# NoahVl/Explaining-In-Style-Reproducibility-Study

Measured on AMD Instinct MI355X. Metric: StylEx G+D+enc train-step images/sec @256px, higher is better.
Workload: dtype bf16; 1 GPU; FFHQ-shaped 256x256 StylEx, batch 32/GPU, GAE=2 (noise+encoder micro-steps), GP every 4th step, ResNet-18 classifier; image_size=256, batch_per_gpu=32, start_step=0, gradient_accumulate_every=2, global_batch=32, parallelism=dp1

## Files before the change

explaining-in-style-reproducibility-study_amd/csrc/fused_bwd.hip:

```cpp
#include <hip/hip_runtime.h>
#include <stdint.h>

#include "stylex_internal.h"

namespace {

constexpr int NT = 256;

template <int K>
struct Acc {
    float4 v[K];
    __device__ __forceinline__ void zero() {
#pragma unroll
        for (int k = 0; k < K; ++k) v[k] = make_float4(0.f, 0.f, 0.f, 0.f);
    }
};

template <int K>
__device__ __forceinline__ void block_reduce_store(Acc<K>& a, float* smem, int cv, int prow, int CV, int rpp, int C,
                                                   float* partial_row , bool active) {
    float4* s4 = reinterpret_cast<float4*>(smem);
    if (active) {
#pragma unroll
        for (int k = 0; k < K; ++k) s4[(k * rpp + prow) * CV + cv] = a.v[k];
    }
    __syncthreads();
    if (active && prow == 0) {
#pragma unroll
        for (int k = 0; k < K; ++k) {
            float4 t = make_float4(0.f, 0.f, 0.f, 0.f);
            for (int r = 0; r < rpp; ++r) {
                float4 u = s4[(k * rpp + r) * CV + cv];
                t.x += u.x; t.y += u.y; t.z += u.z; t.w += u.w;
            }
            float* d = partial_row + (long)k * C + cv * 4;
            if (cv * 4 + 3 < C) {
                *reinterpret_cast<float4*>(d) = t;
            } else {
                float tt[4] = {t.x, t.y, t.z, t.w};
                for (int e = 0; e < 4 && cv * 4 + e < C; ++e) d[e] = tt[e];
            }
        }
    }
}

struct Geo {
    int b, cv, prow, CV, rpp;
    long p_begin, p_end;
    bool active;
};

__device__ __forceinline__ Geo make_geo(int HW, int C, int nchunks) {
    Geo g;
    g.CV = (C + 3) / 4;
    if (g.CV > NT) g.CV = NT;
    g.rpp = NT / g.CV;
    g.cv = threadIdx.x % g.CV;
    g.prow = threadIdx.x / g.CV;
    g.active = g.prow < g.rpp;
    g.b = blockIdx.y;
    long per = ((long)HW + nchunks - 1) / nchunks;
    g.p_begin = (long)blockIdx.x * per;
    g.p_end = g.p_begin + per < HW ? g.p_begin + per : HW;
    return g;
}

__device__ __forceinline__ float4 ld4(const void* p, long off, int bf) { return act_ld4(p, off, bf); }
__device__ __forceinline__ void st4(void* p, long off, float4 v, int bf) { act_st4(p, off, v, bf); }
__device__ __forceinline__ float4 ldp4(const float* p) { return *reinterpret_cast<const float4*>(p); }

__global__ __launch_bounds__(NT) void act_bwd_reduce_kernel(const void* __restrict__ dy, const void* __restrict__ y,
                                                           void* __restrict__ dx, float* __restrict__ partial, int HW,
                                                           int C, int nchunks, int lrelu, float scale, int bf) {
    extern __shared__ __attribute__((aligned(16))) float smem[];
    Geo g = make_geo(HW, C, nchunks);
    Acc<1> a;
    a.zero();
    const int c = g.cv * 4;
    if (g.active && c < C) {
        const long base = (long)g.b * HW;
        for (long p = g.p_begin + g.prow; p < g.p_end; p += g.rpp) {
            const long o = (base + p) * C + c;
            float4 gv = ld4(dy, o, bf);
            gv.x *= scale; gv.y *= scale; gv.z *= scale; gv.w *= scale;
            if (lrelu) {
                const float slope = lrelu == 2 ? 0.f : 0.2f;
                float4 yv = ld4(y, o, bf);
                gv.x = yv.x > 0.f ? gv.x : slope * gv.x;
                gv.y = yv.y > 0.f ? gv.y : slope * gv.y;
                gv.z = yv.z > 0.f ? gv.z : slope * gv.z;
                gv.w = yv.w > 0.f ? gv.w : slope * gv.w;
            }
// ... 62 lines not shown
    extern __shared__ __attribute__((aligned(16))) float smem[];
    Geo g = make_geo(HW, C, nchunks);
    Acc<1> a;
    a.zero();
    const int c = g.cv * 4;
    if (g.active && c < C) {
        float4 s4 = ldp4(s + (long)g.b * C + c);
        const long base = (long)g.b * HW;
        for (long p = g.p_begin + g.prow; p < g.p_end; p += g.rpp) {
            const long o = (base + p) * C + c;
            float4 tv = ld4(t, o, bf);
            float4 xv = ld4(x, o, bf);
            a.v[0].x += xv.x * tv.x; a.v[0].y += xv.y * tv.y; a.v[0].z += xv.z * tv.z; a.v[0].w += xv.w * tv.w;
            if (gx) {
                tv.x *= s4.x; tv.y *= s4.y; tv.z *= s4.z; tv.w *= s4.w;
                st4(gx, o, tv, bf);
            }
        }
    }
    block_reduce_store<1>(a, smem, g.cv, g.prow, g.CV, g.rpp, C, partial + ((long)g.b * nchunks + blockIdx.x) * C,
                          g.active && c < C);
}

inline size_t reduce_smem(int C, int K) {
    int CV = (C + 3) / 4;
    if (CV > NT) CV = NT;
    int rpp = NT / CV;
    return (size_t)K * rpp * CV * 16;
}

inline bool ok_shape(const int64_t* sh, int nchunks) {
    return sh[0] > 0 && sh[1] > 0 && sh[2] > 0 && sh[3] > 0 && sh[3] <= 1024 && (sh[3] % 4 == 0) && nchunks > 0 &&
           sh[0] <= 65535;
}

}

extern "C" {

int stylex_reduce_chunks(const int64_t* sh) {
    long HW = (long)sh[1] * sh[2];
    long n = (2048 + sh[0] - 1) / sh[0];
    long maxc = (HW + 63) / 64;
    if (n > maxc) n = maxc;
    if (n < 1) n = 1;
    return (int)n;
}

int stylex_act_bwd_reduce(const void* dy, const void* y, void* dx, float* partial, const int64_t* sh, int nchunks,
                          int lrelu, float scale, int act_dtype, void* stream) {
    if (act_dtype != 0 && act_dtype != 1) return STYLEX_EINVAL;
    if (!dy || !partial || !ok_shape(sh, nchunks) || (lrelu && !y)) return STYLEX_EINVAL;
    int HW = (int)(sh[1] * sh[2]), C = (int)sh[3];
    hipLaunchKernelGGL(act_bwd_reduce_kernel, dim3(nchunks, (unsigned)sh[0]), dim3(NT), reduce_smem(C, 1),
                       (hipStream_t)stream, dy, y, dx, partial, HW, C, nchunks, lrelu, scale, act_dtype);
    return (int)hipGetLastError();
}

// ... 44 lines not shown
```

explaining-in-style-reproducibility-study_amd/stylex/hip_backend.py:

```python
import os as _os

if _os.environ.get("STYLEX_MIOPEN_ALLOW_BWD_GTC", "0") != "1":
    _os.environ.setdefault("MIOPEN_DEBUG_CONV_IMPLICIT_GEMM_ASM_BWD_GTC_XDLOPS_NHWC", "0")

import atexit
import ctypes
import os
import weakref

import torch

_HERE = os.path.dirname(os.path.abspath(__file__))
LIB_PATH = os.path.join(os.path.dirname(_HERE), "libstylex_hip.so")

F32, BF16, BF16_ACT = 0, 1, 2
EPI_BIAS, EPI_LRELU, EPI_OSCALE, EPI_NOISE, EPI_RESIDUAL, EPI_RELU, EPI_GATE, EPI_NOISE_NAT = 1, 2, 4, 8, 16, 32, 64, 128
EPI_MASK_OUT, EPI_GATE_MASK = 256, 512

_c_f = ctypes.c_void_p
_i64p = ctypes.POINTER(ctypes.c_int64)


class ConvEpilogue(ctypes.Structure):
    _fields_ = [
# ... 42 lines not shown
    "stylex_fold_weight_grad_s2d": (ctypes.c_int, [_c_f, _c_f, _i64p, ctypes.c_void_p]),
    "stylex_conv2d_bwd_weight_s2d_supported": (ctypes.c_int, [_i64p, ctypes.c_int, ctypes.c_int]),
    "stylex_conv2d_bwd_weight_s2d": (ctypes.c_int, [ctypes.c_void_p, ctypes.c_void_p, _c_f, ctypes.c_void_p, ctypes.c_int64, _i64p,
                                                    ctypes.c_int, ctypes.c_float, ctypes.c_int, ctypes.c_int, ctypes.c_void_p]),
    "stylex_upsample2x_bilinear_fwd": (ctypes.c_int, [_c_f, _c_f, _i64p, ctypes.c_int, ctypes.c_void_p]),
    "stylex_upsample2x_bilinear_bwd": (ctypes.c_int, [_c_f, _c_f, _i64p, ctypes.c_int, ctypes.c_void_p]),
    "stylex_rgb_up_blur_add_fwd": (ctypes.c_int, [_c_f, _c_f, _c_f, _i64p, ctypes.c_int, ctypes.c_void_p]),
    "stylex_rgb_up_blur_add_bwd": (ctypes.c_int, [_c_f, _c_f, _i64p, ctypes.c_int, ctypes.c_void_p]),
    "stylex_blur3x3_reflect_fwd": (ctypes.c_int, [_c_f, _c_f, _i64p, ctypes.c_int, ctypes.c_void_p]),
    "stylex_blur3x3_reflect_bwd": (ctypes.c_int, [_c_f, _c_f, _i64p, ctypes.c_int, ctypes.c_void_p]),
    "stylex_bias_act_fwd": (ctypes.c_int, [_c_f, _c_f, _c_f, ctypes.c_int64, _c_f, _c_f, _c_f, _i64p, ctypes.c_int,
                                           ctypes.c_void_p]),
    "stylex_bias_act_bwd": (ctypes.c_int, [_c_f, _c_f, _c_f, _i64p, ctypes.c_int, ctypes.c_void_p]),
    "stylex_rowwise_sumsq": (ctypes.c_int, [_c_f, _c_f, _i64p, ctypes.c_void_p]),
    "stylex_reduce_chunks": (ctypes.c_int, [_i64p]),
    "stylex_act_bwd_reduce": (ctypes.c_int, [_c_f, _c_f, _c_f, _c_f, _i64p, ctypes.c_int, ctypes.c_int, ctypes.c_float,
                                             ctypes.c_int, ctypes.c_void_p]),
    "stylex_modconv_bwd_prep": (ctypes.c_int, [_c_f, _c_f, _c_f, ctypes.c_int64, _c_f, _c_f, _c_f, _c_f, _i64p,
                                               ctypes.c_int, ctypes.c_int, ctypes.c_int, ctypes.c_void_p]),
    "stylex_modconv_bwd_prep_scaled": (ctypes.c_int, [_c_f, _c_f, _c_f, ctypes.c_int64, _c_f, _c_f, _c_f, _c_f, _c_f, _i64p,
                                                      ctypes.c_int, ctypes.c_int, ctypes.c_int, ctypes.c_void_p]),
    "stylex_scale_reduce": (ctypes.c_int, [_c_f, _c_f, _c_f, _c_f, _c_f, _i64p, ctypes.c_int, ctypes.c_int,
                                           ctypes.c_void_p]),
    "stylex_pad_rgb8": (ctypes.c_int, [_c_f, _c_f, _i64p, _i64p, ctypes.c_int, ctypes.c_void_p]),
    "stylex_affine_act_nchw_fwd": (ctypes.c_int, [_c_f, _c_f, _c_f, _c_f, _c_f, ctypes.c_int64, ctypes.c_int64, ctypes.c_int64,
                                                  ctypes.c_int, ctypes.c_void_p]),
    "stylex_affine_act_nchw_bwd": (ctypes.c_int, [_c_f, _c_f, _c_f, _c_f, _c_f, ctypes.c_int64, ctypes.c_int64, ctypes.c_int64,
                                                  ctypes.c_int, ctypes.c_void_p]),
    "stylex_affine_relu_maxpool_fwd": (ctypes.c_int, [_c_f, _c_f, _c_f, _c_f, _c_f, ctypes.c_int64, ctypes.c_int64,
                                                      ctypes.c_int64, ctypes.c_int64, ctypes.c_void_p]),
    "stylex_affine_relu_maxpool_bwd": (ctypes.c_int, [_c_f, _c_f, _c_f, _c_f, ctypes.c_int64, ctypes.c_int64, ctypes.c_int64,
                                                      ctypes.c_int64, ctypes.c_void_p]),
    "stylex_lpips_tap_nhwc_fwd": (ctypes.c_int, [_c_f, _c_f, _c_f, _c_f, _c_f, _c_f, ctypes.c_int64, ctypes.c_int64, ctypes.c_int64,
                                                 ctypes.c_int64, ctypes.c_void_p]),
    "stylex_lpips_tap_nhwc_bwd": (ctypes.c_int, [_c_f, _c_f, _c_f, _c_f, _c_f, _c_f, _c_f, _c_f, ctypes.c_int64, ctypes.c_int64,
                                                 ctypes.c_int64, ctypes.c_void_p]),
    "stylex_nchw_f32_to_nhwc_bf16": (ctypes.c_int, [_c_f, _c_f, ctypes.c_int64, ctypes.c_int64, ctypes.c_int64, ctypes.c_int,
                                                    ctypes.c_void_p]),
    "stylex_nhwc_bf16_to_nchw_f32": (ctypes.c_int, [_c_f, _c_f, _c_f, ctypes.c_int64, ctypes.c_int64, ctypes.c_int64, ctypes.c_void_p]),
    "stylex_resize_norm_fwd": (ctypes.c_int, [_c_f, _c_f, _c_f, _c_f, _i64p, _i64p, ctypes.c_void_p]),
    "stylex_resize_norm_bwd": (ctypes.c_int, [_c_f, _c_f, _c_f, _i64p, ctypes.c_void_p]),
    "stylex_relu_gate_add": (ctypes.c_int, [_c_f, _c_f, _c_f, _c_f, ctypes.c_int64, ctypes.c_void_p]),
    "stylex_maxpool3s2_nhwc_fwd": (ctypes.c_int, [_c_f, _c_f, _c_f, _i64p, ctypes.c_void_p]),
    "stylex_maxpool3s2_nhwc_bwd": (ctypes.c_int, [_c_f, _c_f, _c_f, _i64p, ctypes.c_void_p]),
    "stylex_conv_image_grad": (ctypes.c_int, [_c_f, _c_f, _c_f, _i64p, ctypes.c_void_p]),
    "stylex_lpips_tap_fwd": (ctypes.c_int, [_c_f, _c_f, _c_f, _c_f, _c_f, _c_f, ctypes.c_int64, ctypes.c_int64, ctypes.c_int64,
# ... 1368 lines not shown
                                           _ptr(partial), shp, nch, lr, _adt(gy), _stream()), "stylex_modconv_bwd_prep")
    else:
        gz_scale = _f32(gz_scale)
        _check(lib.stylex_modconv_bwd_prep_scaled(_ptr(gy), _ptr(y), _ptr(noise), ns, _ptr(noise_w), _ptr(noise_b),
                                                  _ptr(gz_scale), _ptr(gz), _ptr(partial), shp, nch, lr, _adt(gy), _stream()),
               "stylex_modconv_bwd_prep_scaled")
    return gz, partial.sum(dim=1)


def scale_reduce(x, t, s, want_gx=True):
    lib = _ensure_device(x)
    assert is_cl(x) and is_cl(t) and x.dtype == t.dtype
    b, c, h, w = x.shape
    shp = _shape(b, h, w, c)
    nch = lib.stylex_reduce_chunks(shp)
    partial = _empty((b, nch, c), dtype=torch.float32, device=x.device)
    gx = empty_cl(tuple(x.shape), x) if want_gx else None
    s = _f32(s)
    _check(lib.stylex_scale_reduce(_ptr(x), _ptr(t), _ptr(s), _ptr(gx), _ptr(partial), shp, nch, _adt(x), _stream()),
           "stylex_scale_reduce")
    return gx, partial.sum(dim=1)


def torgb_ok(x):
    c = x.shape[1]
    if os.environ.get("STYLEX_TORGB", "1") == "0":
        return False
    return x.is_cuda and x.dtype == torch.bfloat16 and 8 <= c <= 512 and (c & (c - 1)) == 0


def torgb_fwd(x, s1, w):
    lib = _ensure_device(x)
    assert is_cl(x) and x.dtype == torch.bfloat16
    b, c, h, wd = x.shape
    y = empty_cl((b, 4, h, wd), x)
    s1, w = _f32(s1), _f32(w)
    _check(lib.stylex_torgb_fwd(_ptr(x), _ptr(s1), _ptr(w), _ptr(y), _shape(b, h, wd, c), _stream()), "stylex_torgb_fwd")
    return y


def torgb_bwd(x, gy, s1, w, want_gx=True):
    lib = _ensure_device(x)
    assert is_cl(x) and is_cl(gy) and gy.shape[1] == 4 and x.dtype == gy.dtype == torch.bfloat16
    b, c, h, wd = x.shape
    shp = _shape(b, h, wd, c)
    nch = lib.stylex_torgb_chunks(shp)
    partial = _empty((b, nch, 3, c), dtype=torch.float32, device=x.device)
    gx = empty_cl(tuple(x.shape), x) if want_gx else None
# ... 76 lines not shown
```

explaining-in-style-reproducibility-study_amd/stylex/networks.py:

```python
import atexit
import math
from math import log2

import os

import torch
import torch.nn.functional as F
from torch import nn

import ops


def exists(v):
    return v is not None


_SIDE = {}
atexit.register(_SIDE.clear)


def _side_stream(t, which=0):
    import os

    if not t.is_cuda or os.environ.get("STYLEX_STREAMS", "1") == "0":
# ... 83 lines not shown

class Conv2DMod(nn.Module):
    def __init__(self, in_chan, out_chan, kernel, demod=True, stride=1, dilation=1, eps=1e-8, **kwargs):
        super().__init__()
        assert stride == 1 and dilation == 1, "only the configuration the reference uses is implemented"
        self.filters, self.demod, self.kernel = out_chan, demod, kernel
        self.stride, self.dilation, self.eps = stride, dilation, eps
        self.weight = nn.Parameter(torch.randn((out_chan, in_chan, kernel, kernel)))
        nn.init.kaiming_normal_(self.weight, a=0, mode="fan_in", nonlinearity="leaky_relu")

    def forward(self, x, y):
        return ops.modulated_conv2d(x, y, self.weight, demod=self.demod, eps=self.eps)


class RGBBlock(nn.Module):
    def __init__(self, latent_dim, input_channel, upsample, rgba=False):
        super().__init__()
        self.input_channel = input_channel
        self.to_style = nn.Linear(latent_dim, input_channel)
        self.conv = Conv2DMod(input_channel, 4 if rgba else 3, 1, demod=False)
        self.upsample = nn.Sequential(Upsample2x(), Blur()) if upsample else None

    def forward(self, x, prev_rgb, istyle, style=None, padded=False):
        style = self.to_style(istyle) if style is None else style
        if padded and not self.conv.demod:
            fused = ops.rgb_block(x, prev_rgb, style, self.conv.weight, exists(self.upsample))
            if fused is not None:
                return fused
        if exists(prev_rgb) and prev_rgb.shape[1] == 4 and self.conv.weight.shape[0] == 3:
            prev_rgb = prev_rgb[:, :3]
        x = self.conv(x, style)
        if exists(prev_rgb):
            x = x + prev_rgb
        if exists(self.upsample):
            x = self.upsample(x)
        return x


class GeneratorBlock(nn.Module):
    def __init__(self, latent_dim, input_channels, filters, upsample=True, upsample_rgb=True, rgba=False):
        super().__init__()
        self.input_channels, self.filters = input_channels, filters
        self.num_style_coords = input_channels + filters
        self.upsample = Upsample2x() if upsample else None
        self.to_style1 = nn.Linear(latent_dim, input_channels)
        self.to_noise1 = nn.Linear(1, filters)
        self.conv1 = Conv2DMod(input_channels, filters, 3)
        self.to_style2 = nn.Linear(latent_dim, filters)
        self.to_noise2 = nn.Linear(1, filters)
        self.conv2 = Conv2DMod(filters, filters, 3)
        self.activation = leaky_relu()
        self.to_rgb = RGBBlock(latent_dim, filters, upsample_rgb, rgba)

    def forward_main(self, x, istyle, inoise, styles=None):
        if exists(self.upsample):
            x = self.upsample(x)
        coords = None
        self._rgb_style = None
        if styles is None:
            fused = ops.style_affines(istyle, self.to_style1, self.to_style2, self.to_rgb.to_style, self.__dict__.setdefault("_aff_cache", {}))
            if fused is not None:
                style1, style2, self._rgb_style, coords = fused
            else:
                style1, style2 = self.to_style1(istyle), self.to_style2(istyle)
        else:
            style1, style2 = styles
        x = ops.modconv_noise_act(x, style1, self.conv1.weight, inoise, self.to_noise1.weight[:, 0],
                                  self.to_noise1.bias, demod=self.conv1.demod, eps=self.conv1.eps)
        x = ops.modconv_noise_act(x, style2, self.conv2.weight, inoise, self.to_noise2.weight[:, 0],
                                  self.to_noise2.bias, demod=self.conv2.demod, eps=self.conv2.eps)
        return x, (coords if coords is not None else torch.cat([style1, style2], dim=-1))

    def forward(self, x, prev_rgb, istyle, inoise):
        x, coords = self.forward_main(x, istyle, inoise)
        rgb = self.to_rgb(x, prev_rgb, istyle, style=self.__dict__.pop("_rgb_style", None))
        return x, rgb, coords


class DiscriminatorBlock(nn.Module):
    def __init__(self, input_channels, filters, downsample=True):
        super().__init__()
        self.conv_res = HipConv2d(input_channels, filters, 1, stride=(2 if downsample else 1))
        self.net = nn.Sequential(HipConv2d(input_channels, filters, 3, padding=1, act=True), _FusedAct(),
                                 HipConv2d(filters, filters, 3, padding=1, act=True), _FusedAct())
        self.downsample = nn.Sequential(Blur(), HipConv2d(filters, filters, 3, padding=1, stride=2)) if downsample else None

    def forward(self, x):
        fused = getattr(ops.impl(), "dblock", None)
        if fused is not None:
# ... 98 lines not shown
```

explaining-in-style-reproducibility-study_amd/stylex/ops.py:

```python
import math

import os

import torch
from contextlib import nullcontext as _nullcontext
import torch.nn.functional as F

import hip_backend as hb

_PRECISION = hb.F32


_NAMES = {"fp32": hb.F32, "f32": hb.F32, "bf16": hb.BF16_ACT, "bf16_f32act": hb.BF16}


def set_precision(name):
    global _PRECISION
    _PRECISION = _NAMES[name]


def get_precision():
    return {hb.F32: "fp32", hb.BF16_ACT: "bf16", hb.BF16: "bf16_f32act"}[_PRECISION]


# ... 523 lines not shown
    @torch.autograd.function.once_differentiable
    def backward(ctx, gy):
        x, s1, w = ctx.saved_tensors
        gx, t = hb.torgb_bwd(x, _cl(gy), s1, w, want_gx=ctx.needs_input_grad[0])
        gs1 = gw = None
        if ctx.needs_input_grad[1]:
            gs1 = (t * w.reshape(1, 3, -1).float()).sum(dim=1)
        if ctx.needs_input_grad[2]:
            gw = (t * s1.float()[:, None, :]).sum(dim=0).reshape(w.shape).to(w.dtype)
        return gx, gs1, gw


class _RGBTailFast(torch.autograd.Function):

    @staticmethod
    def forward(ctx, rgb, prev):
        return hb.rgb_up_blur_add_fwd(_cl(rgb), _cl(prev) if prev is not None else None)

    @staticmethod
    @torch.autograd.function.once_differentiable
    def backward(ctx, gy):
        g = hb.rgb_up_blur_add_bwd(_cl(gy))
        return g, (g if ctx.needs_input_grad[1] else None)


class _BlurS2D(torch.autograd.Function):

    @staticmethod
    def forward(ctx, x):
        return hb.blur3x3_s2d_fwd(_cl(x))

    @staticmethod
    def backward(ctx, gy2):
        return _BlurS2DBwd.apply(gy2)


class _BlurS2DBwd(torch.autograd.Function):
    @staticmethod
    def forward(ctx, gy2):
        return hb.blur3x3_s2d_bwd(_cl(gy2))

    @staticmethod
    def backward(ctx, ggx):
        return _BlurS2D.apply(ggx)


# ... 419 lines not shown
        return _BiasAct.apply(_act(x + n), None)

    @staticmethod
    def upsample2x(x):
        return _Up.apply(_act(x))

    @staticmethod
    def blur3x3(x):
        return _Blur.apply(_act(x))

    @staticmethod
    def blur_down(x, weight, bias, residual, res_scale):
        b, c, h, w = x.shape
        if (_PRECISION != hb.F32 and c % 64 == 0 and weight.shape[0] % 4 == 0 and h % 2 == 0
                and w % 2 == 0 and w // 2 >= 16 and h // 2 >= 16 and tuple(weight.shape[2:]) == (3, 3)):
            x2 = _BlurS2D.apply(_act(x))
            if fast_enabled():
                return _DownS2DFast.apply(x2, weight, bias, _act(residual), res_scale)
            return _ConvBiasActDD.apply(x2, weight, bias, _act(residual), 1, 1, False, res_scale, c)
        return HipOps.conv2d(HipOps.blur3x3(x), weight, bias, stride=2, padding=1, residual=residual,
                             res_scale=res_scale)

    @staticmethod
    def rgb_block(x, prev_rgb, style, weight, upsample):
        if not fast_enabled() or os.environ.get("STYLEX_RGB_TAIL", "1") == "0":
            return None
        x = _act(x)
        if tuple(weight.shape[2:]) != (1, 1) or weight.shape[0] != 3 or not hb.torgb_ok(x):
            return None
        if prev_rgb is not None and (prev_rgb.shape[1] != 4 or prev_rgb.dtype != x.dtype):
            return None
        rgb = _ToRGBFast.apply(x, style + 1, weight)
        if upsample:
            return _RGBTailFast.apply(rgb, prev_rgb)
        return rgb if prev_rgb is None else rgb + prev_rgb

    @staticmethod
    def residual_merge(x, res):
        return (x + res) * (1 / math.sqrt(2))

    @staticmethod
    def dblock(x, conv_res, conv1, conv2, down):
        if not fast_enabled() or os.environ.get("STYLEX_DBLOCK", "1") == "0":
            return None
        if conv1.weight.shape[0] % 4 != 0:
            return None
        return _DBlockFast.apply(x, conv_res.weight, conv_res.bias, conv1.weight, conv1.bias, conv2.weight, conv2.bias,
                                 down.weight if down is not None else None, down.bias if down is not None else None,
                                 down is not None)

    @staticmethod
    def rowwise_sumsq(x2d):
        return _RowSumSq.apply(x2d)


_IMPL = HipOps


def use_impl(impl):
    global _IMPL
    prev = _IMPL
    _IMPL = impl
    return prev


def impl():
    return _IMPL


class _EqualLinearFast(torch.autograd.Function):

    @staticmethod
# ... 149 lines not shown
```

include/stylex_hip.h:

```cpp
#ifndef STYLEX_HIP_H
#define STYLEX_HIP_H

#include <stdint.h>

#ifdef __cplusplus
extern "C" {
#endif

#define STYLEX_F32 0
#define STYLEX_BF16 1
#define STYLEX_BF16_ACT 2

#define STYLEX_EINVAL (-1)
#define STYLEX_EWORKSPACE (-2)

#define STYLEX_CONV_NSHAPE 11

#define STYLEX_EPI_BIAS 1
#define STYLEX_EPI_LRELU 2
#define STYLEX_EPI_OSCALE 4
#define STYLEX_EPI_NOISE 8
#define STYLEX_EPI_RESIDUAL 16
#define STYLEX_EPI_RELU 32
#define STYLEX_EPI_NOISE_NAT 128
// ... 116 lines not shown
                              int64_t C, int64_t HW, int64_t partial_stride, void* stream);
int stylex_lpips_tap_nhwc_bwd(const void* f0, const void* f1, const float* lin, const float* r0, const float* r1, const float* gout,
                              void* g0, void* g1, int64_t B, int64_t C, int64_t HW, void* stream);

int stylex_weight_sumsq(const float* w, float* wsq, int64_t O, int64_t C, int64_t K, void* stream);
int stylex_modcoeff_fwd(const float* style, const float* wsq, float* s1, float* d, int64_t B, int64_t C, int64_t O,
                        float eps, void* stream);
int stylex_modcoeff_bwd(const float* gd, const float* d, const float* s1, const float* wsq, const float* w,
                        const float* gs1, float* gstyle, float* gw, int64_t B, int64_t C, int64_t O, int64_t K,
                        void* stream);

int stylex_reduce_chunks(const int64_t* shape);
int stylex_act_bwd_reduce(const void* dy, const void* y, void* dx, float* partial, const int64_t* shape, int nchunks,
                          int lrelu, float scale, int act_dtype, void* stream);
int stylex_modconv_bwd_prep(const void* gy, const void* y, const float* noise, int64_t noise_stride,
                            const float* noise_w, const float* noise_b, void* gz, float* partial,
                            const int64_t* shape, int nchunks, int lrelu, int act_dtype, void* stream);
int stylex_modconv_bwd_prep_scaled(const void* gy, const void* y, const float* noise, int64_t noise_stride,
                                   const float* noise_w, const float* noise_b, const float* gz_scale, void* gz,
                                   float* partial, const int64_t* shape, int nchunks, int lrelu, int act_dtype,
                                   void* stream);
int stylex_scale_reduce(const void* x, const void* t, const float* s, void* gx, float* partial, const int64_t* shape,
                        int nchunks, int act_dtype, void* stream);

int stylex_torgb_chunks(const int64_t* shape);
int stylex_torgb_fwd(const void* x, const float* s1, const float* w, void* y, const int64_t* shape, void* stream);
int stylex_torgb_bwd(const void* x, const void* gy, const float* s1, const float* w, void* gx, float* partial,
                     const int64_t* shape, void* stream);

int stylex_timing_enable(int on);
int stylex_timing_pause(int on);
int stylex_timing_report(int kernel_class, int64_t* launches, double* total_ms, double* total_flops,
                         double* total_bytes);
int stylex_timing_layers(int64_t* meta, double* vals, int64_t cap);
int stylex_timing_kernels(char* names, int64_t* meta, double* vals, int64_t cap);

#define STYLEX_ADAM_COPY_PACK 0
#define STYLEX_ADAM_COPY_PACK_S2D 1
#define STYLEX_ADAM_COPY_SUMSQ 2
typedef struct {
    float* p;
    const float* g;
    float* m;
    float* v;
    const float* step;
    int64_t numel;
// ... 32 lines not shown
```

Before: 992.0 images/sec.

## Fuse StyleGAN generator block forward/backward into custom autograd with fused backward kernels

Adds a fused generator-block autograd function that runs upsample, two modulated convs with noise/lrelu epilogues, and toRGB in one unit. Its backward uses two new HIP kernels that fold the RGB gradient, the incoming gradient sum, the lrelu backward, the noise weight/bias reductions and the demod-coefficient reductions into single passes over activations. The per-strip reduction helpers move into a shared header. This aims to cut separate elementwise and reduction kernels and repeated activation reads in generator backward, at the cost of saving more intermediates and adding extra code paths with shape guards.

```diff
diff --git a/explaining-in-style-reproducibility-study_amd/csrc/fused_bwd.hip b/explaining-in-style-reproducibility-study_amd/csrc/fused_bwd.hip
--- a/explaining-in-style-reproducibility-study_amd/csrc/fused_bwd.hip
+++ b/explaining-in-style-reproducibility-study_amd/csrc/fused_bwd.hip
@@ -2,72 +2,11 @@
 #include <stdint.h>
 
 #include "stylex_internal.h"
+#include "strip_reduce.h"
 
 namespace {
 
-constexpr int NT = 256;
-
-template <int K>
-struct Acc {
-    float4 v[K];
-    __device__ __forceinline__ void zero() {
-#pragma unroll
-        for (int k = 0; k < K; ++k) v[k] = make_float4(0.f, 0.f, 0.f, 0.f);
-    }
-};
-
-template <int K>
-__device__ __forceinline__ void block_reduce_store(Acc<K>& a, float* smem, int cv, int prow, int CV, int rpp, int C,
-                                                   float* partial_row , bool active) {
-    float4* s4 = reinterpret_cast<float4*>(smem);
-    if (active) {
-#pragma unroll
-        for (int k = 0; k < K; ++k) s4[(k * rpp + prow) * CV + cv] = a.v[k];
-    }
-    __syncthreads();
-    if (active && prow == 0) {
-#pragma unroll
-        for (int k = 0; k < K; ++k) {
-            float4 t = make_float4(0.f, 0.f, 0.f, 0.f);
-            for (int r = 0; r < rpp; ++r) {
-                float4 u = s4[(k * rpp + r) * CV + cv];
-                t.x += u.x; t.y += u.y; t.z += u.z; t.w += u.w;
-            }
-            float* d = partial_row + (long)k * C + cv * 4;
-            if (cv * 4 + 3 < C) {
-                *reinterpret_cast<float4*>(d) = t;
-            } else {
-                float tt[4] = {t.x, t.y, t.z, t.w};
-                for (int e = 0; e < 4 && cv * 4 + e < C; ++e) d[e] = tt[e];
-            }
-        }
-    }
-}
-
-struct Geo {
-    int b, cv, prow, CV, rpp;
-    long p_begin, p_end;
-    bool active;
-};
-
-__device__ __forceinline__ Geo make_geo(int HW, int C, int nchunks) {
-    Geo g;
-    g.CV = (C + 3) / 4;
-    if (g.CV > NT) g.CV = NT;
-    g.rpp = NT / g.CV;
-    g.cv = threadIdx.x % g.CV;
-    g.prow = threadIdx.x / g.CV;
-    g.active = g.prow < g.rpp;
-    g.b = blockIdx.y;
-    long per = ((long)HW + nchunks - 1) / nchunks;
-    g.p_begin = (long)blockIdx.x * per;
-    g.p_end = g.p_begin + per < HW ? g.p_begin + per : HW;
-    return g;
-}
-
-__device__ __forceinline__ float4 ld4(const void* p, long off, int bf) { return act_ld4(p, off, bf); }
-__device__ __forceinline__ void st4(void* p, long off, float4 v, int bf) { act_st4(p, off, v, bf); }
-__device__ __forceinline__ float4 ldp4(const float* p) { return *reinterpret_cast<const float4*>(p); }
+using namespace stylex_strip;
 
 __global__ __launch_bounds__(NT) void act_bwd_reduce_kernel(const void* __restrict__ dy, const void* __restrict__ y,
                                                            void* __restrict__ dx, float* __restrict__ partial, int HW,
@@ -176,18 +115,6 @@
                           g.active && c < C);
 }
 
-inline size_t reduce_smem(int C, int K) {
-    int CV = (C + 3) / 4;
-    if (CV > NT) CV = NT;
-    int rpp = NT / CV;
-    return (size_t)K * rpp * CV * 16;
-}
-
-inline bool ok_shape(const int64_t* sh, int nchunks) {
-    return sh[0] > 0 && sh[1] > 0 && sh[2] > 0 && sh[3] > 0 && sh[3] <= 1024 && (sh[3] % 4 == 0) && nchunks > 0 &&
-           sh[0] <= 65535;
-}
-
 }
 
 extern "C" {
diff --git a/explaining-in-style-reproducibility-study_amd/csrc/gblock_bwd.hip b/explaining-in-style-reproducibility-study_amd/csrc/gblock_bwd.hip
--- /dev/null
+++ b/explaining-in-style-reproducibility-study_amd/csrc/gblock_bwd.hip
@@ -0,0 +1,231 @@
+#include <hip/hip_runtime.h>
+#include <stdint.h>
+
+#include "stylex_internal.h"
+#include "strip_reduce.h"
+
+namespace {
+
+using namespace stylex_strip;
+
+__device__ __forceinline__ float4 rnd4(float4 v, int bf) { return bf ? act_unpack4(act_pack4(v)) : v; }
+
+__device__ __forceinline__ float noise_at(const float* noise, int ns, int natural, int b, int p, int W) {
+    const int h = p / W, w = p - h * W;
+    return natural ? noise[((long)b * ns + h) * ns + w] : noise[((long)b * ns + w) * ns + h];
+}
+
+__device__ __forceinline__ void prep_step(float4 gv, float4 yv, float nz, float4 w4, float4 b4, float4 d4, int lrelu,
+                                          bool scaled, void* gz, long o, int bf, float4* a) {
+    float4 t = yv;
+    if (lrelu) {
+        gv.x = yv.x > 0.f ? gv.x : 0.2f * gv.x; t.x = yv.x > 0.f ? yv.x : 5.f * yv.x;
+        gv.y = yv.y > 0.f ? gv.y : 0.2f * gv.y; t.y = yv.y > 0.f ? yv.y : 5.f * yv.y;
+        gv.z = yv.z > 0.f ? gv.z : 0.2f * gv.z; t.z = yv.z > 0.f ? yv.z : 5.f * yv.z;
+        gv.w = yv.w > 0.f ? gv.w : 0.2f * gv.w; t.w = yv.w > 0.f ? yv.w : 5.f * yv.w;
+    }
+    if (scaled) st4(gz, o, make_float4(gv.x * d4.x, gv.y * d4.y, gv.z * d4.z, gv.w * d4.w), bf);
+    else st4(gz, o, gv, bf);
+    a[0].x += gv.x * (t.x - (nz * w4.x + b4.x));
+    a[0].y += gv.y * (t.y - (nz * w4.y + b4.y));
+    a[0].z += gv.z * (t.z - (nz * w4.z + b4.z));
+    a[0].w += gv.w * (t.w - (nz * w4.w + b4.w));
+    a[1].x += gv.x * nz; a[1].y += gv.y * nz; a[1].z += gv.z * nz; a[1].w += gv.w * nz;
+    a[2].x += gv.x; a[2].y += gv.y; a[2].z += gv.z; a[2].w += gv.w;
+}
+
+template <bool RGB, bool BF>
+__global__ __launch_bounds__(NT) void gblock_out_bwd_kernel(const void* __restrict__ y, const void* __restrict__ ga,
+                                                           const void* __restrict__ gb, const void* __restrict__ grgb,
+                                                           const float* __restrict__ s_rgb, const float* __restrict__ w_rgb,
+                                                           const float* __restrict__ noise, int ns, int natural,
+                                                           const float* __restrict__ nw, const float* __restrict__ nb,
+                                                           const float* __restrict__ gz_scale, void* __restrict__ gz,
+                                                           float* __restrict__ partial, int H, int W, int C, int nchunks,
+                                                           int lrelu) {
+    extern __shared__ __attribute__((aligned(16))) float smem[];
+    constexpr int K = 3, bf = BF ? 1 : 0;
+    const int HW = H * W;
+    Geo g = make_geo(HW, C, nchunks);
+    Acc<K> a;
+    a.zero();
+    const int c = g.cv * 4;
+    if (g.active && c < C) {
+        float4 w4 = make_float4(0.f, 0.f, 0.f, 0.f), b4 = w4;
+        if (noise) {
+            w4 = ldp4(nw + c);
+            b4 = ldp4(nb + c);
+        }
+        float4 d4 = make_float4(1.f, 1.f, 1.f, 1.f);
+        if (gz_scale) d4 = ldp4(gz_scale + (long)g.b * C + c);
+        float4 m0 = w4, m1 = w4, m2 = w4;
+        if (RGB) {
+            const float4 s4 = ldp4(s_rgb + (long)g.b * C + c);
+            const float4 r0 = ldp4(w_rgb + c), r1 = ldp4(w_rgb + C + c), r2 = ldp4(w_rgb + 2 * C + c);
+            m0 = make_float4(r0.x * s4.x, r0.y * s4.y, r0.z * s4.z, r0.w * s4.w);
+            m1 = make_float4(r1.x * s4.x, r1.y * s4.y, r1.z * s4.z, r1.w * s4.w);
+            m2 = make_float4(r2.x * s4.x, r2.y * s4.y, r2.z * s4.z, r2.w * s4.w);
+        }
+        const long base = (long)g.b * HW;
+        constexpr int UNR = RGB ? 1 : 2;
+        for (long p0 = g.p_begin + g.prow; p0 < g.p_end; p0 += UNR * g.rpp) {
+            float4 yv[UNR], av[UNR], bv[UNR], qv[UNR];
+            float nz[UNR];
+#pragma unroll
+            for (int u = 0; u < UNR; ++u) {
+                const long p = p0 + u * g.rpp;
+                if (p >= g.p_end) continue;
+                const long o = (base + p) * C + c;
+                yv[u] = ld4(y, o, bf);
+                if (ga) av[u] = ld4(ga, o, bf);
+                if (gb) bv[u] = ld4(gb, o, bf);
+                if (RGB) qv[u] = ld4(grgb, (base + p) * 4, bf);
+                nz[u] = noise ? noise_at(noise, ns, natural, g.b, (int)p, W) : 0.f;
+            }
+#pragma unroll
+            for (int u = 0; u < UNR; ++u) {
+                const long p = p0 + u * g.rpp;
+                if (p >= g.p_end) continue;
+                float4 gv = make_float4(0.f, 0.f, 0.f, 0.f);
+                bool have = false;
+                if (ga) {
+                    gv = av[u];
+                    have = true;
+                }
+                if (gb) {
+                    gv = have ? rnd4(make_float4(gv.x + bv[u].x, gv.y + bv[u].y, gv.z + bv[u].z, gv.w + bv[u].w), bf) : bv[u];
+                    have = true;
+                }
+                if (RGB) {
+                    const float g0 = qv[u].x, g1 = qv[u].y, g2 = qv[u].z;
+                    float4 r;
+                    r.x = fmaf(g2, m2.x, fmaf(g0, m0.x, g1 * m1.x));
+                    r.y = fmaf(g2, m2.y, fmaf(g0, m0.y, g1 * m1.y));
+                    r.z = fmaf(g2, m2.z, fmaf(g0, m0.z, g1 * m1.z));
+                    r.w = fmaf(g2, m2.w, fmaf(g0, m0.w, g1 * m1.w));
+                    r = rnd4(r, bf);
+                    gv = have ? rnd4(make_float4(gv.x + r.x, gv.y + r.y, gv.z + r.z, gv.w + r.w), bf) : r;
+                }
+                prep_step(gv, yv[u], nz[u], w4, b4, d4, lrelu, gz_scale != nullptr, gz, (base + p) * C + c, bf, a.v);
+            }
+        }
+    }
+    block_reduce_store<K>(a, smem, g.cv, g.prow, g.CV, g.rpp, C, partial + ((long)g.b * nchunks + blockIdx.x) * K * C,
+                          g.active && c < C);
+}
+
+template <bool BF>
+__global__ __launch_bounds__(NT) void gblock_mid_bwd_kernel(const void* __restrict__ y, const void* __restrict__ t,
+                                                           const float* __restrict__ s, const float* __restrict__ noise,
+                                                           int ns, int natural, const float* __restrict__ nw,
+                                                           const float* __restrict__ nb, const float* __restrict__ gz_scale,
+                                                           void* __restrict__ gz, float* __restrict__ partial,
+                                                           float* __restrict__ partial2, int H, int W, int C, int nchunks,
+                                                           int lrelu) {
+    extern __shared__ __attribute__((aligned(16))) float smem[];
+    constexpr int bf = BF ? 1 : 0;
+    const int HW = H * W;
+    Geo g = make_geo(HW, C, nchunks);
+    Acc<4> a;
+    a.zero();
+    const int c = g.cv * 4;
+    if (g.active && c < C) {
+        float4 w4 = make_float4(0.f, 0.f, 0.f, 0.f), b4 = w4;
+        if (noise) {
+            w4 = ldp4(nw + c);
+            b4 = ldp4(nb + c);
+        }
+        float4 d4 = make_float4(1.f, 1.f, 1.f, 1.f);
+        if (gz_scale) d4 = ldp4(gz_scale + (long)g.b * C + c);
+        const float4 s4 = ldp4(s + (long)g.b * C + c);
+        const long base = (long)g.b * HW;
+        for (long p0 = g.p_begin + g.prow; p0 < g.p_end; p0 += 2 * g.rpp) {
+            float4 tv[2], yv[2];
+            float nz[2];
+#pragma unroll
+            for (int u = 0; u < 2; ++u) {
+                const long p = p0 + u * g.rpp;
+                if (p >= g.p_end) continue;
+                const long o = (base + p) * C + c;
+                tv[u] = ld4(t, o, bf);
+                yv[u] = ld4(y, o, bf);
+                nz[u] = noise ? noise_at(noise, ns, natural, g.b, (int)p, W) : 0.f;
+            }
+#pragma unroll
+            for (int u = 0; u < 2; ++u) {
+                const long p = p0 + u * g.rpp;
+                if (p >= g.p_end) continue;
+                float4 tt = tv[u];
+                const float4 yy = yv[u];
+                a.v[3].x += yy.x * tt.x; a.v[3].y += yy.y * tt.y; a.v[3].z += yy.z * tt.z; a.v[3].w += yy.w * tt.w;
+                tt.x *= s4.x; tt.y *= s4.y; tt.z *= s4.z; tt.w *= s4.w;
+                prep_step(rnd4(tt, bf), yy, nz[u], w4, b4, d4, lrelu, gz_scale != nullptr, gz, (base + p) * C + c, bf, a.v);
+            }
+        }
+    }
+    const long row = (long)g.b * nchunks + blockIdx.x;
+    block_reduce_store<4>(a, smem, g.cv, g.prow, g.CV, g.rpp, C, partial + row * 3 * C, g.active && c < C,
+                          partial2 + row * C, 3);
+}
+
+inline bool aligned16(const void* p) { return (reinterpret_cast<uintptr_t>(p) & 15) == 0; }
+
+inline bool noise_ok(const float* noise, int64_t ns, const float* nw, const float* nb, const int64_t* sh) {
+    return !noise || (nw && nb && aligned16(nw) && aligned16(nb) && ns >= sh[1] && ns >= sh[2] && ns <= INT32_MAX);
+}
+
+}
+
+extern "C" {
+
+int stylex_gblock_out_bwd(const void* y2, const void* g_a, const void* g_b, const void* g_rgb, const float* s_rgb,
+                          const float* w_rgb, const float* noise, int64_t noise_stride, int noise_natural,
+                          const float* noise_w, const float* noise_b, const float* d2, void* gz2, float* partial,
+                          const int64_t* sh, int nchunks, int lrelu, int act_dtype, void* stream) {
+    if (act_dtype != 0 && act_dtype != 1) return STYLEX_EINVAL;
+    if (!y2 || !gz2 || !partial || !sh || !ok_shape(sh, nchunks)) return STYLEX_EINVAL;
+    const bool rgb = g_rgb != nullptr;
+    if (rgb != (s_rgb != nullptr) || rgb != (w_rgb != nullptr)) return STYLEX_EINVAL;
+    if (!g_a && !g_b && !rgb) return STYLEX_EINVAL;
+    if (!noise_ok(noise, noise_stride, noise_w, noise_b, sh)) return STYLEX_EINVAL;
+    if (!aligned16(y2) || !aligned16(g_a) || !aligned16(g_b) || !aligned16(g_rgb) || !aligned16(s_rgb) ||
+        !aligned16(w_rgb) || !aligned16(d2) || !aligned16(gz2) || !aligned16(partial))
+        return STYLEX_EINVAL;
+    if (sh[1] * sh[2] > INT32_MAX) return STYLEX_EINVAL;
+    const int C = (int)sh[3];
+    const dim3 grid(nchunks, (unsigned)sh[0]);
+#define GBLOCK_OUT(RGB_, BF_)                                                                                             \
+    hipLaunchKernelGGL((gblock_out_bwd_kernel<RGB_, BF_>), grid, dim3(NT), reduce_smem(C, 3),                   \
+                       (hipStream_t)stream, y2, g_a, g_b, g_rgb, s_rgb, w_rgb, noise, (int)noise_stride, noise_natural,  \
+                       noise_w, noise_b, d2, gz2, partial, (int)sh[1], (int)sh[2], C, nchunks, lrelu)
+    if (rgb && act_dtype) GBLOCK_OUT(true, true);
+    else if (rgb) GBLOCK_OUT(true, false);
+    else if (act_dtype) GBLOCK_OUT(false, true);
+    else GBLOCK_OUT(false, false);
+#undef GBLOCK_OUT
+    return (int)hipGetLastError();
+}
+
+int stylex_gblock_mid_bwd(const void* y1, const void* t2, const float* s2, const float* noise, int64_t noise_stride,
+                          int noise_natural, const float* noise_w, const float* noise_b, const float* d1, void* gz1,
+                          float* partial, float* partial_s, const int64_t* sh, int nchunks, int lrelu, int act_dtype,
+                          void* stream) {
+    if (act_dtype != 0 && act_dtype != 1) return STYLEX_EINVAL;
+    if (!y1 || !t2 || !s2 || !gz1 || !partial || !partial_s || !sh || !ok_shape(sh, nchunks)) return STYLEX_EINVAL;
+    if (!noise_ok(noise, noise_stride, noise_w, noise_b, sh)) return STYLEX_EINVAL;
+    if (!aligned16(y1) || !aligned16(t2) || !aligned16(s2) || !aligned16(d1) || !aligned16(gz1) || !aligned16(partial) ||
+        !aligned16(partial_s))
+        return STYLEX_EINVAL;
+    if (sh[1] * sh[2] > INT32_MAX) return STYLEX_EINVAL;
+    const int C = (int)sh[3];
+#define GBLOCK_MID(BF_)                                                                                                  \
+    hipLaunchKernelGGL(gblock_mid_bwd_kernel<BF_>, dim3(nchunks, (unsigned)sh[0]), dim3(NT), reduce_smem(C, 4),            \
+                       (hipStream_t)stream, y1, t2, s2, noise, (int)noise_stride, noise_natural, noise_w, noise_b, d1, gz1, \
+                       partial, partial_s, (int)sh[1], (int)sh[2], C, nchunks, lrelu)
+    if (act_dtype) GBLOCK_MID(true);
+    else GBLOCK_MID(false);
+#undef GBLOCK_MID
+    return (int)hipGetLastError();
+}
+
+}
diff --git a/explaining-in-style-reproducibility-study_amd/csrc/strip_reduce.h b/explaining-in-style-reproducibility-study_amd/csrc/strip_reduce.h
--- /dev/null
+++ b/explaining-in-style-reproducibility-study_amd/csrc/strip_reduce.h
@@ -0,0 +1,86 @@
+#pragma once
+#include <hip/hip_runtime.h>
+#include <stdint.h>
+
+#include "stylex_internal.h"
+
+namespace stylex_strip {
+
+constexpr int NT = 256;
+
+template <int K>
+struct Acc {
+    float4 v[K];
+    __device__ __forceinline__ void zero() {
+#pragma unroll
+        for (int k = 0; k < K; ++k) v[k] = make_float4(0.f, 0.f, 0.f, 0.f);
+    }
+};
+
+template <int K>
+__device__ __forceinline__ void block_reduce_store(Acc<K>& a, float* smem, int cv, int prow, int CV, int rpp, int C,
+                                                   float* partial_row , bool active,
+                                                   float* partial_row2 = nullptr, int k2 = K) {
+    float4* s4 = reinterpret_cast<float4*>(smem);
+    if (active) {
+#pragma unroll
+        for (int k = 0; k < K; ++k) s4[(k * rpp + prow) * CV + cv] = a.v[k];
+    }
+    __syncthreads();
+    if (active && prow == 0) {
+#pragma unroll
+        for (int k = 0; k < K; ++k) {
+            float4 t = make_float4(0.f, 0.f, 0.f, 0.f);
+            for (int r = 0; r < rpp; ++r) {
+                float4 u = s4[(k * rpp + r) * CV + cv];
+                t.x += u.x; t.y += u.y; t.z += u.z; t.w += u.w;
+            }
+            float* d = (k < k2 ? partial_row + (long)k * C : partial_row2 + (long)(k - k2) * C) + cv * 4;
+            if (cv * 4 + 3 < C) {
+                *reinterpret_cast<float4*>(d) = t;
+            } else {
+                float tt[4] = {t.x, t.y, t.z, t.w};
+                for (int e = 0; e < 4 && cv * 4 + e < C; ++e) d[e] = tt[e];
+            }
+        }
+    }
+}
+
+struct Geo {
+    int b, cv, prow, CV, rpp;
+    long p_begin, p_end;
+    bool active;
+};
+
+__device__ __forceinline__ Geo make_geo(int HW, int C, int nchunks) {
+    Geo g;
+    g.CV = (C + 3) / 4;
+    if (g.CV > NT) g.CV = NT;
+    g.rpp = NT / g.CV;
+    g.cv = threadIdx.x % g.CV;
+    g.prow = threadIdx.x / g.CV;
+    g.active = g.prow < g.rpp;
+    g.b = blockIdx.y;
+    long per = ((long)HW + nchunks - 1) / nchunks;
+    g.p_begin = (long)blockIdx.x * per;
+    g.p_end = g.p_begin + per < HW ? g.p_begin + per : HW;
+    return g;
+}
+
+__device__ __forceinline__ float4 ld4(const void* p, long off, int bf) { return act_ld4(p, off, bf); }
+__device__ __forceinline__ void st4(void* p, long off, float4 v, int bf) { act_st4(p, off, v, bf); }
+__device__ __forceinline__ float4 ldp4(const float* p) { return *reinterpret_cast<const float4*>(p); }
+
+inline size_t reduce_smem(int C, int K) {
+    int CV = (C + 3) / 4;
+    if (CV > NT) CV = NT;
+    int rpp = NT / CV;
+    return (size_t)K * rpp * CV * 16;
+}
+
+inline bool ok_shape(const int64_t* sh, int nchunks) {
+    return sh[0] > 0 && sh[1] > 0 && sh[2] > 0 && sh[3] > 0 && sh[3] <= 1024 && (sh[3] % 4 == 0) && nchunks > 0 &&
+           sh[0] <= 65535;
+}
+
+}
diff --git a/explaining-in-style-reproducibility-study_amd/stylex/hip_backend.py b/explaining-in-style-reproducibility-study_amd/stylex/hip_backend.py
--- a/explaining-in-style-reproducibility-study_amd/stylex/hip_backend.py
+++ b/explaining-in-style-reproducibility-study_amd/stylex/hip_backend.py
@@ -88,6 +88,10 @@
                                                       ctypes.c_int, ctypes.c_int, ctypes.c_int, ctypes.c_void_p]),
     "stylex_scale_reduce": (ctypes.c_int, [_c_f, _c_f, _c_f, _c_f, _c_f, _i64p, ctypes.c_int, ctypes.c_int,
                                            ctypes.c_void_p]),
+    "stylex_gblock_out_bwd": (ctypes.c_int, [_c_f] * 7 + [ctypes.c_int64, ctypes.c_int] + [_c_f] * 5 + [_i64p, ctypes.c_int,
+                                             ctypes.c_int, ctypes.c_int, ctypes.c_void_p]),
+    "stylex_gblock_mid_bwd": (ctypes.c_int, [_c_f] * 4 + [ctypes.c_int64, ctypes.c_int] + [_c_f] * 6 + [_i64p, ctypes.c_int,
+                                             ctypes.c_int, ctypes.c_int, ctypes.c_void_p]),
     "stylex_pad_rgb8": (ctypes.c_int, [_c_f, _c_f, _i64p, _i64p, ctypes.c_int, ctypes.c_void_p]),
     "stylex_affine_act_nchw_fwd": (ctypes.c_int, [_c_f, _c_f, _c_f, _c_f, _c_f, ctypes.c_int64, ctypes.c_int64, ctypes.c_int64,
                                                   ctypes.c_int, ctypes.c_void_p]),
@@ -1502,8 +1506,56 @@
     return gx, partial.sum(dim=1)
 
 
-def torgb_ok(x):
-    c = x.shape[1]
+def _noise_args(noise, noise_nat, noise_w, noise_b):
+    plane = _f32(noise_nat if noise_nat is not None else noise)
+    if plane is None:
+        return None, 0, 0, None, None
+    assert plane.dim() == 3 and plane.shape[1] == plane.shape[2]
+    return plane, plane.shape[1], int(noise_nat is not None), _f32(noise_w), _f32(noise_b)
+
+
+def gblock_out_bwd(y2, g_a, g_b, g_rgb, s_rgb, w_rgb, noise, noise_w, noise_b, lrelu, d2=None, noise_nat=None):
+    lib = _ensure_device(y2)
+    assert is_cl(y2) and all(g is None or (is_cl(g) and g.dtype == y2.dtype and g.shape == y2.shape) for g in (g_a, g_b))
+    b, c, h, w = y2.shape
+    shp = _shape(b, h, w, c)
+    nch = lib.stylex_reduce_chunks(shp)
+    partial = _empty((b, nch, 3, c), dtype=torch.float32, device=y2.device)
+    if g_rgb is not None:
+        assert is_cl(g_rgb) and g_rgb.dtype == y2.dtype and tuple(g_rgb.shape) == (b, 4, h, w)
+        s_rgb, w_rgb = _f32(s_rgb), _f32(w_rgb)
+        assert tuple(s_rgb.shape) == (b, c) and w_rgb.numel() == 3 * c
+    else:
+        s_rgb = w_rgb = None
+    gz = empty_cl(tuple(y2.shape), y2)
+    plane, ns, nat, noise_w, noise_b = _noise_args(noise, noise_nat, noise_w, noise_b)
+    d2 = _f32(d2)
+    _check(lib.stylex_gblock_out_bwd(_ptr(y2), _ptr(g_a), _ptr(g_b), _ptr(g_rgb), _ptr(s_rgb), _ptr(w_rgb), _ptr(plane), ns, nat,
+                                     _ptr(noise_w), _ptr(noise_b), _ptr(d2), _ptr(gz), _ptr(partial), shp, nch, int(bool(lrelu)),
+                                     _adt(y2), _stream()), "stylex_gblock_out_bwd")
+    return gz, partial.sum(dim=1)
+
+
+def gblock_mid_bwd(y1, t2, s2, noise, noise_w, noise_b, lrelu, d1=None, noise_nat=None):
+    lib = _ensure_device(y1)
+    assert is_cl(y1) and is_cl(t2) and y1.dtype == t2.dtype and y1.shape == t2.shape
+    b, c, h, w = y1.shape
+    shp = _shape(b, h, w, c)
+    nch = lib.stylex_reduce_chunks(shp)
+    partial = _empty((b, nch, 3, c), dtype=torch.float32, device=y1.device)
+    partial_s = _empty((b, nch, c), dtype=torch.float32, device=y1.device)
+    gz = empty_cl(tuple(y1.shape), y1)
+    plane, ns, nat, noise_w, noise_b = _noise_args(noise, noise_nat, noise_w, noise_b)
+    s2, d1 = _f32(s2), _f32(d1)
+    assert tuple(s2.shape) == (b, c)
+    _check(lib.stylex_gblock_mid_bwd(_ptr(y1), _ptr(t2), _ptr(s2), _ptr(plane), ns, nat, _ptr(noise_w), _ptr(noise_b), _ptr(d1),
+                                     _ptr(gz), _ptr(partial), _ptr(partial_s), shp, nch, int(bool(lrelu)), _adt(y1), _stream()),
+           "stylex_gblock_mid_bwd")
+    return gz, partial.sum(dim=1), partial_s.sum(dim=1)
+
+
+def torgb_ok(x, channels=None):
+    c = x.shape[1] if channels is None else channels
     if os.environ.get("STYLEX_TORGB", "1") == "0":
         return False
     return x.is_cuda and x.dtype == torch.bfloat16 and 8 <= c <= 512 and (c & (c - 1)) == 0
diff --git a/explaining-in-style-reproducibility-study_amd/stylex/networks.py b/explaining-in-style-reproducibility-study_amd/stylex/networks.py
--- a/explaining-in-style-reproducibility-study_amd/stylex/networks.py
+++ b/explaining-in-style-reproducibility-study_amd/stylex/networks.py
@@ -129,14 +129,17 @@
         self.upsample = nn.Sequential(Upsample2x(), Blur()) if upsample else None
 
     def forward(self, x, prev_rgb, istyle, style=None, padded=False):
-        style = self.to_style(istyle) if style is None else style
+        pre = self.__dict__.pop("_pre", None)
+        pre = pre[1] if pre is not None and pre[0] is x else None
+        if pre is None:
+            style = self.to_style(istyle) if style is None else style
         if padded and not self.conv.demod:
-            fused = ops.rgb_block(x, prev_rgb, style, self.conv.weight, exists(self.upsample))
+            fused = ops.rgb_block(x, prev_rgb, style, self.conv.weight, exists(self.upsample), **({} if pre is None else {"pre": pre}))
             if fused is not None:
                 return fused
         if exists(prev_rgb) and prev_rgb.shape[1] == 4 and self.conv.weight.shape[0] == 3:
             prev_rgb = prev_rgb[:, :3]
-        x = self.conv(x, style)
+        x = self.conv(x, style) if pre is None else pre[:, :3]
         if exists(prev_rgb):
             x = x + prev_rgb
         if exists(self.upsample):
@@ -160,10 +163,9 @@
         self.to_rgb = RGBBlock(latent_dim, filters, upsample_rgb, rgba)
 
     def forward_main(self, x, istyle, inoise, styles=None):
-        if exists(self.upsample):
-            x = self.upsample(x)
         coords = None
         self._rgb_style = None
+        self.to_rgb.__dict__.pop("_pre", None)
         if styles is None:
             fused = ops.style_affines(istyle, self.to_style1, self.to_style2, self.to_rgb.to_style, self.__dict__.setdefault("_aff_cache", {}))
             if fused is not None:
@@ -172,6 +174,17 @@
                 style1, style2 = self.to_style1(istyle), self.to_style2(istyle)
         else:
             style1, style2 = styles
+        fused = getattr(ops.impl(), "gblock", None) if exists(self.upsample) else None
+        if fused is not None:
+            out = fused(x, style1, style2, self.conv1, self.conv2, inoise, self.to_noise1, self.to_noise2,
+                        rgb_style=self._rgb_style, rgb_conv=self.to_rgb.conv)
+            if out is not None:
+                x, rgb = out
+                if rgb is not None:
+                    self.to_rgb._pre = (x, rgb)
+                return x, (coords if coords is not None else torch.cat([style1, style2], dim=-1))
+        if exists(self.upsample):
+            x = self.upsample(x)
         x = ops.modconv_noise_act(x, style1, self.conv1.weight, inoise, self.to_noise1.weight[:, 0],
                                   self.to_noise1.bias, demod=self.conv1.demod, eps=self.conv1.eps)
         x = ops.modconv_noise_act(x, style2, self.conv2.weight, inoise, self.to_noise2.weight[:, 0],
diff --git a/explaining-in-style-reproducibility-study_amd/stylex/ops.py b/explaining-in-style-reproducibility-study_amd/stylex/ops.py
--- a/explaining-in-style-reproducibility-study_amd/stylex/ops.py
+++ b/explaining-in-style-reproducibility-study_amd/stylex/ops.py
@@ -569,6 +569,56 @@
     def backward(ctx, gy):
         g = hb.rgb_up_blur_add_bwd(_cl(gy))
         return g, (g if ctx.needs_input_grad[1] else None)
+
+
+class _GBlockFast(torch.autograd.Function):
+
+    @staticmethod
+    def forward(ctx, x, s1, d1, w1, s2, d2, w2, noise, noise_nat, nw1, nb1, nw2, nb2, s_rgb, w_rgb):
+        x_up = hb.upsample2x_fwd(_cl(x))
+        nat_fwd = noise_nat is not None and noise_nat.shape[1] % 4 == 0
+        epi = dict(noise=noise_nat, noise_natural=True) if nat_fwd else dict(noise=noise)
+        y1 = hb.conv2d_fwd(x_up, w1, 1, 1, _PRECISION, in_scale=s1, out_scale=d1, noise_w=nw1, noise_b=nb1, lrelu=True, **epi)
+        y2 = hb.conv2d_fwd(y1, w2, 1, 1, _PRECISION, in_scale=s2, out_scale=d2, noise_w=nw2, noise_b=nb2, lrelu=True, **epi)
+        rgb = hb.torgb_fwd(y2, s_rgb, w_rgb) if s_rgb is not None else None
+        ctx.save_for_backward(x_up, y1, y2, s1, d1, w1, s2, d2, w2, noise, noise_nat, nw1, nb1, nw2, nb2, s_rgb, w_rgb)
+        ctx.set_materialize_grads(False)
+        return y2, rgb
+
+    @staticmethod
+    @torch.autograd.function.once_differentiable
+    def backward(ctx, g_y2, g_rgb):
+        x_up, y1, y2, s1, d1, w1, s2, d2, w2, noise, nat, nw1, nb1, nw2, nb2, s_rgb, w_rgb = ctx.saved_tensors
+        need = ctx.needs_input_grad
+        if s_rgb is None:
+            g_rgb = None
+        if g_y2 is None and g_rgb is None:
+            return (None,) * 15
+        fold = _PRECISION != hb.F32 and os.environ.get("STYLEX_FOLD_D", "1") != "0"
+        g_rgb = _cl(g_rgb) if g_rgb is not None else None
+        gz2, sums2 = hb.gblock_out_bwd(y2, _cl(g_y2) if g_y2 is not None else None, None, g_rgb, s_rgb, w_rgb, noise, nw2, nb2,
+                                       True, d2=d2 if fold else None, noise_nat=nat)
+        gd2 = sums2[:, 0] / d2
+        gnw2, gnb2 = sums2[:, 1:3].sum(0)
+        gs_rgb = gw_rgb = None
+        if g_rgb is not None and (need[13] or need[14]):
+            t_rgb = hb.torgb_bwd(y2, g_rgb, s_rgb, w_rgb, want_gx=False)[1]
+            if need[13]:
+                gs_rgb = (t_rgb * w_rgb.reshape(1, 3, -1).float()).sum(dim=1)
+            if need[14]:
+                gw_rgb = (t_rgb * s_rgb.float()[:, None, :]).sum(dim=0).reshape(w_rgb.shape).to(w_rgb.dtype)
+        t2 = hb.conv2d_bwd_data(gz2, w2, tuple(y1.shape), 1, 1, _PRECISION, **({} if fold else dict(in_scale=d2)))
+        gw2 = hb.conv2d_bwd_weight(y1, gz2, tuple(w2.shape), 1, 1, _PRECISION, x_scale=s2,
+                                   dy_scale=None if fold else d2) if need[6] else None
+        gz1, sums1, gs2 = hb.gblock_mid_bwd(y1, t2, s2, noise, nw1, nb1, True, d1=d1 if fold else None, noise_nat=nat)
+        gd1 = sums1[:, 0] / d1
+        gnw1, gnb1 = sums1[:, 1:3].sum(0)
+        t1 = hb.conv2d_bwd_data(gz1, w1, tuple(x_up.shape), 1, 1, _PRECISION, **({} if fold else dict(in_scale=d1)))
+        gw1 = hb.conv2d_bwd_weight(x_up, gz1, tuple(w1.shape), 1, 1, _PRECISION, x_scale=s1,
+                                   dy_scale=None if fold else d1) if need[3] else None
+        gx_up, gs1 = hb.scale_reduce(x_up, t1, s1, want_gx=need[0])
+        gx = hb.upsample2x_bwd(gx_up) if need[0] else None
+        return gx, gs1, gd1, gw1, gs2, gd2, gw2, None, None, gnw1, gnb1, gnw2, gnb2, gs_rgb, gw_rgb
 
 
 class _BlurS2D(torch.autograd.Function):
@@ -1034,7 +1084,7 @@
                              res_scale=res_scale)
 
     @staticmethod
-    def rgb_block(x, prev_rgb, style, weight, upsample):
+    def rgb_block(x, prev_rgb, style, weight, upsample, pre=None):
         if not fast_enabled() or os.environ.get("STYLEX_RGB_TAIL", "1") == "0":
             return None
         x = _act(x)
@@ -1042,7 +1092,7 @@
             return None
         if prev_rgb is not None and (prev_rgb.shape[1] != 4 or prev_rgb.dtype != x.dtype):
             return None
-        rgb = _ToRGBFast.apply(x, style + 1, weight)
+        rgb = _ToRGBFast.apply(x, style + 1, weight) if pre is None else pre
         if upsample:
             return _RGBTailFast.apply(rgb, prev_rgb)
         return rgb if prev_rgb is None else rgb + prev_rgb
@@ -1060,6 +1110,28 @@
         return _DBlockFast.apply(x, conv_res.weight, conv_res.bias, conv1.weight, conv1.bias, conv2.weight, conv2.bias,
                                  down.weight if down is not None else None, down.bias if down is not None else None,
                                  down is not None)
+
+    @staticmethod
+    def gblock(x, style1, style2, conv1, conv2, inoise, to_noise1, to_noise2, rgb_style=None, rgb_conv=None):
+        if not fast_enabled() or os.environ.get("STYLEX_GBLOCK", "1") == "0" or not x.is_cuda:
+            return None
+        w1, w2 = conv1.weight, conv2.weight
+        if not (conv1.demod and conv2.demod and tuple(w1.shape[2:]) == (3, 3) and tuple(w2.shape[2:]) == (3, 3)):
+            return None
+        if not (_reducible(w1.shape[0]) and _reducible(w1.shape[1]) and w2.shape[0] == w2.shape[1] == w1.shape[0]):
+            return None
+        if 2 * x.shape[2] <= 8 or 2 * x.shape[3] <= 8 or inoise.shape[1] != inoise.shape[2]:
+            return None
+        x = _act(x)
+        s1, d1 = mod_coeffs(style1, w1, True, conv1.eps)
+        s2, d2 = mod_coeffs(style2, w2, True, conv2.eps)
+        nat = _natural_noise(inoise) if os.environ.get("STYLEX_NOISE_NAT", "1") != "0" else None
+        s_rgb = w_rgb = None
+        if (rgb_conv is not None and rgb_style is not None and not rgb_conv.demod and tuple(rgb_conv.weight.shape[1:]) ==
+                (w2.shape[0], 1, 1) and rgb_conv.weight.shape[0] == 3 and hb.torgb_ok(x, channels=w2.shape[0])):
+            s_rgb, w_rgb = rgb_style + 1, rgb_conv.weight
+        return _GBlockFast.apply(x, s1, d1, w1, s2, d2, w2, inoise[:, :, :, 0], nat, to_noise1.weight[:, 0], to_noise1.bias,
+                                 to_noise2.weight[:, 0], to_noise2.bias, s_rgb, w_rgb)
 
     @staticmethod
     def rowwise_sumsq(x2d):
diff --git a/include/stylex_hip.h b/include/stylex_hip.h
--- a/include/stylex_hip.h
+++ b/include/stylex_hip.h
@@ -162,6 +162,15 @@
                                    void* stream);
 int stylex_scale_reduce(const void* x, const void* t, const float* s, void* gx, float* partial, const int64_t* shape,
                         int nchunks, int act_dtype, void* stream);
+
+int stylex_gblock_out_bwd(const void* y2, const void* g_a, const void* g_b, const void* g_rgb, const float* s_rgb,
+                          const float* w_rgb, const float* noise, int64_t noise_stride, int noise_natural,
+                          const float* noise_w, const float* noise_b, const float* d2, void* gz2, float* partial,
+                          const int64_t* shape, int nchunks, int lrelu, int act_dtype, void* stream);
+int stylex_gblock_mid_bwd(const void* y1, const void* t2, const float* s2, const float* noise, int64_t noise_stride,
+                          int noise_natural, const float* noise_w, const float* noise_b, const float* d1, void* gz1,
+                          float* partial, float* partial_s, const int64_t* shape, int nchunks, int lrelu, int act_dtype,
+                          void* stream);
 
 int stylex_torgb_chunks(const int64_t* shape);
 int stylex_torgb_fwd(const void* x, const float* s1, const float* w, void* y, const int64_t* shape, void* stream);
```

After: 1004 images/sec, median of 6. 1.01x the previous value.
